# bhavyageethika/multimodal_autonomous_driving_perception_and_planning

Hardware: AMD Instinct MI355X
Metric: end-to-end frames/sec (1280x720 synthetic) (higher is better)
Workload: dtype f64; 1 GPU; config4: 64 stream(s)/GPU x 1-frame window per step, 1280x720, simulated detection + IoU tracker + 6-state KF + 21-candidate planner, one launch per step, up to 4 consecutive steps in flight; streams_per_gpu=64, window=1, graph=False, taggers=False, allgather_track_tables=False, fused_step=True, overlapped_steps=4, steps_per_library_call=8, parallelism=stream-sharded x1

## Files before the change

multimodal_autonomous_driving_perception_and_planning_amd/csrc/kf.hip:

```cpp
#include "common.h"

namespace {

struct KfOut {
    double v[AV_VSTATE_DOUBLES];
};

struct Filter {
    double x[6];
    double P[6][6];
    double prev_heading, prev_speed, time;
};

__device__ __forceinline__ void extract(Filter& k, double dt, KfOut& o) {
    const double vx = k.x[2], vy = k.x[3];
    const double speed = sqrt(vx * vx + vy * vy);
    const double heading = speed > 0.1 ? atan2(vy, vx) : k.prev_heading;
    const double acc = dt > 0.0 ? (speed - k.prev_speed) / dt : 0.0;
    double dh = heading - k.prev_heading;
    const double pi = 3.141592653589793;
    if (dh > pi) dh -= 2.0 * pi;
    else if (dh < -pi) dh += 2.0 * pi;
    const double yaw = dt > 0.0 ? dh / dt : 0.0;
    o.v[0] = k.x[0], o.v[1] = k.x[1], o.v[2] = vx, o.v[3] = vy;
// ... 110 lines not shown
    double* st = kf_state + (size_t)s * AV_KF_STATE_DOUBLES;

    bool bad = st[45] != 0.0;
    if (lane < 36) {
        const int r = lane / 6, c = lane - r * 6;
        if (((r ^ c) & 1) && st[6 + lane] != 0.0) bad = true;
    }
    if (__ballot(bad) != 0ull) {
        if (lane == 0) st[45] = 1.0;
        return false;
    }
    const int ax = lane & 1;
    Axis a;
    a.x0 = st[ax], a.x1 = st[2 + ax], a.x2 = st[4 + ax];
#pragma unroll
    for (int r = 0; r < 3; ++r)
#pragma unroll
        for (int c = 0; c < 3; ++c) a.p[r][c] = st[6 + (2 * r + ax) * 6 + (2 * c + ax)];
    double carry_h = st[42], carry_sp = st[43], time = st[44];
    double pp[3][3], Kc[3][2] = {{0, 0}, {0, 0}, {0, 0}};
#pragma unroll
    for (int r = 0; r < 3; ++r)
#pragma unroll
        for (int c = 0; c < 3; ++c) pp[r][c] = a.p[r][c];
    bool steady = false;
    __builtin_amdgcn_s_waitcnt(0x0F70);
    const double dt = cfg.dt, h = 0.5 * (dt * dt), q = cfg.process_noise, rr = cfg.measurement_noise;

    for (int f0 = 0; f0 < n_frames; f0 += KF_BATCH) {
        const int nb = (n_frames - f0) < KF_BATCH ? (n_frames - f0) : KF_BATCH;
        const size_t sf0 = (size_t)s * n_frames + f0;
        int m_mine = 0;
        if (lane < nb) {
            const int m = mode ? (int)mode[sf0 + lane] : 1;
            m_mine = m;
            ml[lane] = m;
            double4 zz = make_double4(0.0, 0.0, 0.0, 0.0);
            if (z && (m == 1 || m == 3)) zz = reinterpret_cast<const double4*>(z)[sf0 + lane];
            *reinterpret_cast<double4*>(zl[lane]) = zz;
        }
        __builtin_amdgcn_s_waitcnt(0x0F70);
        __builtin_amdgcn_fence(__ATOMIC_RELEASE, "wavefront", "local");
        __builtin_amdgcn_wave_barrier();
        __builtin_amdgcn_fence(__ATOMIC_ACQUIRE, "wavefront", "local");

        const unsigned long long ones = __ballot(m_mine == 1);
        for (int fb = 0; fb < nb;) {
            if (steady) {
                const double p00 = a.p[0][0], p11 = a.p[1][1];
                while (fb < nb && ((ones >> fb) & 1ull)) {
                    const double zp = zl[fb][ax], zv = zl[fb][2 + ax];
                    const double nx0 = a.x0 + dt * a.x1 + h * a.x2;
                    const double nx1 = a.x1 + dt * a.x2;
                    a.x0 = nx0, a.x1 = nx1;
                    time += dt;
                    const double vpred = a.x1;
                    const double y0 = zp - a.x0, y1 = zv - a.x1;
                    a.x0 = a.x0 + (Kc[0][0] * y0 + Kc[0][1] * y1);
                    a.x1 = a.x1 + (Kc[1][0] * y0 + Kc[1][1] * y1);
                    a.x2 = a.x2 + (Kc[2][0] * y0 + Kc[2][1] * y1);
                    if (lane < 2) {
                        double* w = raw[fb];
                        w[ax] = a.x0, w[2 + ax] = a.x1, w[4 + ax] = vpred;
                        w[6 + ax] = p00, w[8 + ax] = p11;
                        if (lane == 0) w[10] = time, w[11] = 1.0;
                    }
                    ++fb;
                }
                if (fb >= nb) break;
            }
            const int m = ml[fb];
            const double zp = zl[fb][ax], zv = zl[fb][2 + ax];
            double vpred = a.x1;
            {
                if (m != 3) {
                    axis_predict(a, dt, h, q);
                    time += dt;
                    vpred = a.x1;
                }
                if (m == 1 || m == 3) axis_update(a, zp, zv, rr, Kc);
                bool same = m == 1;
#pragma unroll
                for (int r = 0; r < 3; ++r)
#pragma unroll
                    for (int c = 0; c < 3; ++c) same = same && a.p[r][c] == pp[r][c], pp[r][c] = a.p[r][c];
                steady = __ballot(same) == ~0ull;
            }
            if (lane < 2) {
                double* w = raw[fb];
                w[ax] = a.x0, w[2 + ax] = a.x1, w[4 + ax] = vpred;
                w[6 + ax] = a.p[0][0], w[8 + ax] = a.p[1][1];
                if (lane == 0) w[10] = time, w[11] = (double)m;
            }
            ++fb;
        }
        __builtin_amdgcn_fence(__ATOMIC_RELEASE, "wavefront", "local");
        __builtin_amdgcn_wave_barrier();
        __builtin_amdgcn_fence(__ATOMIC_ACQUIRE, "wavefront", "local");

        const bool on = lane < nb;
        const double* w = raw[on ? lane : 0];
        const int m = (int)w[11];
        const double px = w[0], py = w[1], vx = w[2], vy = w[3], vxp = w[4], vyp = w[5];
        const bool has_pred = (m != 3), has_post = (m == 1 || m == 3);
        const double sp_p = sqrt(vxp * vxp + vyp * vyp);
        const double sp_q = sqrt(vx * vx + vy * vy);
        const bool val_p = has_pred && sp_p > 0.1, val_q = has_post && sp_q > 0.1;
        const double at_p = atan2(vyp, vxp), at_q = atan2(vy, vx);
        const bool gives = on && (val_p || val_q);
        const double give_h = val_q ? at_q : at_p;
        const unsigned long long gmask = __ballot(gives);
        const unsigned long long below = gmask & ((1ull << lane) - 1ull);
        const int src = below ? 63 - __clzll((long long)below) : 0;
        const double from_h = __shfl(give_h, src, 64);
        const double h_in = below ? from_h : carry_h;
        const double last_sp = has_post ? sp_q : sp_p;
        double sp_in = __shfl_up(last_sp, 1, 64);
        if (lane == 0) sp_in = carry_sp;
        const double h_p = has_pred ? (val_p ? at_p : h_in) : h_in;
        const double prev_h = has_pred ? h_p : h_in;
        const double prev_s = has_pred ? sp_p : sp_in;
        double heading, speed, ph, ps;
        if (m == 0) heading = h_p, speed = sp_p, ph = h_in, ps = sp_in;
        else if (m == 2) heading = (sp_p > 0.1 ? at_p : prev_h), speed = sp_p, ph = prev_h, ps = prev_s;
        else heading = (val_q ? at_q : prev_h), speed = sp_q, ph = prev_h, ps = prev_s;
        const double acc = dt > 0.0 ? (speed - ps) / dt : 0.0;
        double dh = heading - ph;
        const double pi = 3.141592653589793;
        if (dh > pi) dh -= 2.0 * pi;
        else if (dh < -pi) dh += 2.0 * pi;
        const double yaw = dt > 0.0 ? dh / dt : 0.0;
        if (on) {
            double2* dst = reinterpret_cast<double2*>(out_state + (sf0 + lane) * AV_VSTATE_DOUBLES);
            dst[0] = make_double2(px, py), dst[1] = make_double2(vx, vy), dst[2] = make_double2(heading, speed);
            dst[3] = make_double2(acc, yaw), dst[4] = make_double2(w[10], sqrt(w[6] + w[7]));
            dst[5] = make_double2(sqrt(w[8] + w[9]), 0.0);
            if (plan_state) reinterpret_cast<double4*>(plan_state)[sf0 + lane] = make_double4(px, py, heading, speed);
        }
        carry_h = __shfl(heading, nb - 1, 64);
        carry_sp = __shfl(speed, nb - 1, 64);
    }

    if (lane < 2) {
        st[ax] = a.x0, st[2 + ax] = a.x1, st[4 + ax] = a.x2;
#pragma unroll
        for (int r = 0; r < 3; ++r)
#pragma unroll
            for (int c = 0; c < 3; ++c) st[6 + (2 * r + ax) * 6 + (2 * c + ax)] = a.p[r][c];
        if (lane == 0) st[42] = carry_h, st[43] = carry_sp, st[44] = time;
    }
    return true;
}

template <bool DENSE>
__global__ void __launch_bounds__(64) kf_axis_kernel(av_kf_cfg cfg, int n_frames, const double* __restrict__ z,
                                                     const uint8_t* __restrict__ mode, double* __restrict__ kf_state,
                                                     double* __restrict__ out_state, double* __restrict__ plan_state) {
    __builtin_amdgcn_s_setprio(3);
    const bool separable = kf_axis_body(cfg, n_frames, z, mode, kf_state, out_state, plan_state, blockIdx.x, threadIdx.x);
    if (DENSE && !separable && threadIdx.x == 0) kf_dense_stream_lds(cfg, blockIdx.x, n_frames, z, mode, kf_state, out_state, plan_state);
}

__global__ void kf_reset_kernel(int n_streams, double* kf_state) {
    const int s = blockIdx.x * blockDim.x + threadIdx.x;
    if (s >= n_streams) return;
    double* st = kf_state + (size_t)s * AV_KF_STATE_DOUBLES;
    for (int i = 0; i < AV_KF_STATE_DOUBLES; ++i) st[i] = 0.0;
    for (int i = 0; i < 6; ++i) st[6 + i * 7] = 10.0;
}

}

#ifndef AVHOT_DEVICE_ONLY

extern "C" {

int av_kf_reset(av_ctx* ctx, av_stream_t stream, int n_streams, double* kf_state) {
    AV_REQUIRE(ctx && kf_state && n_streams > 0, AV_EINVAL, "av_kf_reset: bad argument");
    hipLaunchKernelGGL(kf_reset_kernel, dim3((n_streams + 63) / 64), dim3(64), 0, as_stream(stream), n_streams, kf_state);
    AV_LAUNCH_CHECK();
    return AV_OK;
}

int av_kf_step(av_ctx* ctx, av_stream_t stream, const av_kf_cfg* cfg, int n_streams, int n_frames, const double* z,
               const uint8_t* mode, double* kf_state, double* out_state, double* plan_state) {
    AV_REQUIRE(ctx && cfg && kf_state && out_state, AV_EINVAL, "av_kf_step: null argument");
    AV_REQUIRE(z || mode, AV_EINVAL, "av_kf_step: z may only be NULL when every mode is 0 or 2");
    AV_REQUIRE(n_streams > 0 && n_frames > 0, AV_EINVAL, "av_kf_step: n_streams/n_frames must be > 0");
    if (n_frames <= 2) {
        hipLaunchKernelGGL(kf_axis_kernel<true>, dim3(n_streams), dim3(64), 0, as_stream(stream), *cfg, n_frames, z, mode, kf_state,
                           out_state, plan_state);
        AV_LAUNCH_CHECK();
        return AV_OK;
    }
    hipLaunchKernelGGL(kf_axis_kernel<false>, dim3(n_streams), dim3(64), 0, as_stream(stream), *cfg, n_frames, z, mode,
                       kf_state, out_state, plan_state);
    AV_LAUNCH_CHECK();
    hipLaunchKernelGGL(kf_kernel, dim3((n_streams + 63) / 64), dim3(64), 0, as_stream(stream), *cfg, n_streams,
                       n_frames, z, mode, kf_state, out_state, plan_state, 1);
    AV_LAUNCH_CHECK();
    return AV_OK;
}

}

#endif
```

multimodal_autonomous_driving_perception_and_planning_amd/csrc/planner.hip:

```cpp
#include "common.h"

#include <cmath>



namespace {

struct PlanParams {
    int n, n_lat, C;
    double dt, H;
    double w_lat, w_vel, w_acc, w_curv;
    const double *t, *alpha, *q, *dtd, *lat;
    double atq[20];
};

static const double ATAN_Q[20] = {
    -0x1.5555555555549p-2, 0x1.99999999979b9p-3,  -0x1.24924923e22b4p-3, 0x1.c71c718e5a102p-4,
    -0x1.745d120df88fbp-4, 0x1.3b1362fc35ab5p-4,  -0x1.110deef367776p-4, 0x1.e1b3c8d50e91fp-5,
    -0x1.ae2c7119eb922p-5, 0x1.81fdd2525246ap-5,  -0x1.56daf4786fd80p-5, 0x1.2575526b2309ap-5,
    -0x1.d168e01adf666p-6, 0x1.462cc26bda000p-6,  -0x1.8055065b73333p-7, 0x1.693bd6b79999ap-8,
    -0x1.fdf4e15cccccdp-10, 0x1.f224118000000p-12, -0x1.2568700000000p-14, 0x1.2ed799999999ap-18,
};

__device__ __forceinline__ double atan2_fast(double y, double x, const double (&Q)[20]) {
    const double ax = __builtin_fabs(x), ay = __builtin_fabs(y);
    const bool swap = ay > ax;
    const double mx = swap ? ay : ax, mn = swap ? ax : ay;
    double r = __builtin_amdgcn_rcp(mx);
    r = __builtin_fma(__builtin_fma(-mx, r, 1.0), r, r);
    r = __builtin_fma(__builtin_fma(-mx, r, 1.0), r, r);
    double t = mn * r;
    t = __builtin_fma(__builtin_fma(-t, mx, mn), r, t);
    t = mx == 0.0 ? 0.0 : t;
    const double z = t * t;
    double pz = Q[19];
#pragma unroll
    for (int k = 18; k >= 0; --k) pz = __builtin_fma(pz, z, Q[k]);
    double a = __builtin_fma(t * z, pz, t);
    a = swap ? 1.5707963267948966 - a : a;
    a = x < 0.0 ? 3.141592653589793 - a : a;
    return __builtin_copysign(a, y);
}

__host__ __device__ inline int even_up(int v) { return (v + 1) & ~1; }

__host__ __device__ inline size_t plan_lds_doubles(int G, int n, int C, int NW = 4) {
    return (size_t)G * 3 * n * 2 + even_up(G * 3 * 3) + (size_t)G * 8 + (size_t)3 * even_up(G * C) + (size_t)NW * n * 6;
}

__device__ __forceinline__ void wave_lds_fence() {
    __builtin_amdgcn_fence(__ATOMIC_RELEASE, "wavefront", "local");
    __builtin_amdgcn_wave_barrier();
    __builtin_amdgcn_fence(__ATOMIC_ACQUIRE, "wavefront", "local");
}

template <int G, int NW>
__device__ __forceinline__ void plan_block(const PlanParams& p, int f0, int n_states, const double* __restrict__ state,
                                           const double* __restrict__ ref, int n_ref, const double* __restrict__ obs, int n_obs,
                                           double* __restrict__ wp, double* __restrict__ cost, int32_t* __restrict__ order, double* sm) {
    const int n = p.n, C = p.C;
    double* vs = sm;
    double* base = vs + (size_t)G * 3 * n * 2;
    double* trig = base + even_up(G * 3 * 3);
    double* costs = trig + G * 8;
    double* stage_all = costs + 3 * even_up(G * C);
    const int CS = even_up(G * C);

    const int tid = threadIdx.x, lane = tid & 63, wid = tid >> 6;
    double* stage = stage_all + (size_t)wid * n * 6;
    constexpr int P = G * 3;
    static_assert(NW >= 2, "the heading terms take the last wave");

    auto bcast = [&](double x, int i) {
        const unsigned lo = (unsigned)__builtin_amdgcn_readlane((int)(unsigned)__double_as_longlong(x), i);
        const unsigned hi = (unsigned)__builtin_amdgcn_readlane((int)(unsigned)((unsigned long long)__double_as_longlong(x) >> 32), i);
        return __longlong_as_double((long long)(((unsigned long long)hi << 32) | lo));
    };
    auto terms = [&](double v0, double dv, int i, double& v, double& vdt, double& velt, double& acct) {
        v = v0 + dv * p.alpha[i];
        vdt = v * p.dt;
        const double e = v - 10.0;
        velt = p.w_vel * (e * e);
        acct = 0.0;
        if (i > 0) {
            const double vp = v0 + dv * p.alpha[i - 1];
            const double a = (v - vp) / p.dtd[i];
            acct = p.w_acc * (a * a);
        }
    };
    auto cost_chains = [&](double velt, double acct, unsigned long long hasm, double* b) {
        double sv = 0.0;
#pragma unroll
        for (int i = 0; i < 64; ++i)
            if (i < n) sv = sv + bcast(velt, i);
        double run = sv, sa = 0.0;
#pragma unroll
        for (int i = 1; i < 64; ++i)
            if (i < n && ((hasm >> i) & 1ull)) {
                const double term = bcast(acct, i);
                run = run + term, sa = sa + term;
            }
        if (lane == 0) b[0] = sv, b[1] = sa, b[2] = run;
    };

    const bool fast = n <= 64 && P <= NW;
    double k_velt = 0.0, k_acct = 0.0;
    unsigned long long k_has = 0;
    bool k_live = false;
    if (fast) {
        if (wid < P) {
            const int g = wid / 3, k = wid - g * 3, f = f0 + g;
            if (f < n_states) {
                const double v0 = state[(size_t)f * 4 + 3];
                const double vt = 8.0 + 2.0 * (double)k;
                const double dv = vt - v0;
                double* o = vs + ((size_t)(g * 3 + k) * n) * 2;
                double v = 0.0, vdt = 0.0;
                bool has = false;
                if (lane < n) terms(v0, dv, lane, v, vdt, k_velt, k_acct), has = lane > 0 && p.dtd[lane] > 0.0;
                k_has = __ballot(has), k_live = true;
                double sacc = 0.0, my_s = 0.0;
#pragma unroll
                for (int i = 1; i < 64; ++i)
                    if (i < n) {
                        sacc = sacc + bcast(vdt, i);
                        my_s = lane == i ? sacc : my_s;
                    }
                if (lane < n) o[2 * lane] = v, o[2 * lane + 1] = my_s;
            }
        }
    } else {
        for (int pr = wid; pr < P; pr += NW) {
            const int g = pr / 3, k = pr - g * 3, f = f0 + g;
            if (f >= n_states) continue;
            const double v0 = state[(size_t)f * 4 + 3];
            const double vt = 8.0 + 2.0 * (double)k;
            const double dv = vt - v0;
            double* o = vs + ((size_t)(g * 3 + k) * n) * 2;
            double* b = base + (g * 3 + k) * 3;
            double* tv = stage;
            for (int i = lane; i < n; i += 64) {
                double v, vdt, velt, acct;
                terms(v0, dv, i, v, vdt, velt, acct);
                o[2 * i] = v, tv[i] = vdt, tv[n + i] = velt, tv[2 * n + i] = acct;
            }
            wave_lds_fence();
            if (lane == 0) {
                double sacc = 0.0, sv = 0.0;
                o[1] = 0.0;
                sv = sv + tv[n];
                for (int i = 1; i < n; ++i) {
                    sacc = sacc + tv[i];
                    o[2 * i + 1] = sacc;
                    sv = sv + tv[n + i];
                }
                double run = sv, sa = 0.0;
                for (int i = 1; i < n; ++i) {
                    if (p.dtd[i] > 0.0) {
                        const double term = tv[2 * n + i];
                        run = run + term, sa = sa + term;
                    }
                }
                b[0] = sv, b[1] = sa, b[2] = run;
            }
            wave_lds_fence();
        }
    }
    if (wid == NW - 1 && lane < 2 * G) {
        const int g = lane >> 1, f = f0 + g;
        if (f < n_states) {
            const double h0 = state[(size_t)f * 4 + 2];
            double* tg = trig + g * 8;
            double sn, cs;
            if (lane & 1) {
                sincos(h0 + 1.5707963267948966, &sn, &cs);
                tg[4] = cs, tg[5] = sn;
            } else {
                sincos(h0, &sn, &cs);
                tg[0] = state[(size_t)f * 4 + 0], tg[1] = state[(size_t)f * 4 + 1];
                tg[2] = cs, tg[3] = sn, tg[6] = h0;
            }
        }
    }
    __syncthreads();
    if (k_live) cost_chains(k_velt, k_acct, k_has, base + wid * 3);

    const double q_l = lane < n ? p.q[lane] : 0.0, q_l1 = lane + 1 < n ? p.q[lane + 1] : 0.0, t_l = lane < n ? p.t[lane] : 0.0;
    const bool extra = n_ref > 0 || n_obs > 0;
    for (int j = fast ? (wid - P % NW + NW) % NW : wid; j < G * C; j += NW) {
        const int g = j / C, c = j - g * C, f = f0 + g;
        if (f >= n_states) continue;
        const int li = c / 3, k = c - li * 3;
        const double df = p.lat[li];
        const double* tg = trig + g * 8;
        const double x0 = tg[0], y0 = tg[1], cs = tg[2], sn = tg[3], c2 = tg[4], s2 = tg[5], h0 = tg[6];
        const double* o = vs + ((size_t)(g * 3 + k) * n) * 2;

        for (int i = lane; i < n; i += 64) {
            const double v = o[2 * i], s = o[2 * i + 1];
            const bool first = i == lane;
            const double d = df * (first ? q_l : p.q[i]);
            double x = x0 + s * cs, y = y0 + s * sn;
            x = x + d * c2, y = y + d * s2;
            double hd = 0.0;
            if (i < n - 1) {
                const double s1 = o[2 * i + 3], d1 = df * (first ? q_l1 : p.q[i + 1]);
                double x1 = x0 + s1 * cs, y1 = y0 + s1 * sn;
                x1 = x1 + d1 * c2, y1 = y1 + d1 * s2;
                hd = atan2_fast(y1 - y, x1 - x, p.atq);
            }
            double* w = stage + (size_t)i * 6;
            w[0] = x, w[1] = y, w[2] = hd, w[3] = v, w[4] = first ? t_l : p.t[i], w[5] = 0.0;
        }
        wave_lds_fence();
        double lat_sum = 0.0, curv_sum = 0.0, obs_sum = 0.0;
        for (int i = lane; i < n; i += 64) {
            double* w = stage + (size_t)i * 6;
            double curv = 0.0;
            if (i > 0 && i < n - 1) {
                const double hp = stage[(size_t)(i - 1) * 6 + 2];
                curv = (w[2] - hp) / (w[3] * p.dt + 1e-6);
                w[5] = curv;
            }
            curv_sum += p.w_curv * (curv * curv);
            const double x = w[0], y = w[1];
            if (n_ref > 0) {
                double md = INFINITY;
                for (int r = 0; r < n_ref; ++r) {
                    const double dx = ref[2 * r] - x, dy = ref[2 * r + 1] - y;
                    const double dd = sqrt(dx * dx + dy * dy);
                    md = dd < md ? dd : md;
                }
                lat_sum += p.w_lat * (md * md);
            }
            for (int q = 0; q < n_obs; ++q) {
                const double ox = obs[3 * q], oy = obs[3 * q + 1], rad = obs[3 * q + 2];
                const double ex = x - ox, ey = y - oy;
                const double dist = sqrt(ex * ex + ey * ey);
                if (dist < rad * 2.0) obs_sum += 1000.0 * (rad * 2.0 - dist);
                else if (dist < rad * 4.0) obs_sum += 10.0 / (dist - rad + 0.1);
            }
        }
        wave_lds_fence();
        if (lane == 0) stage[(size_t)(n - 1) * 6 + 2] = n > 1 ? stage[(size_t)(n - 2) * 6 + 2] : h0;
        curv_sum = wave_sum_dpp(curv_sum);
        if (extra) lat_sum = wave_sum_dpp(lat_sum), obs_sum = wave_sum_dpp(obs_sum);
        if (lane == 0) costs[g * C + c] = lat_sum, costs[CS + g * C + c] = curv_sum, costs[2 * CS + g * C + c] = obs_sum;
        wave_lds_fence();
        if (wp) {
            const double2* src = reinterpret_cast<const double2*>(stage);
            double2* dst = reinterpret_cast<double2*>(wp + ((size_t)f * C + c) * n * 6);
            for (int q = lane; q < n * 3; q += 64) dst[q] = src[q];
        }
        wave_lds_fence();
    }
    __syncthreads();

    for (int idx = tid; idx < G * C; idx += NW * 64) {
        const int g = idx / C, c = idx - g * C, k = c % 3;
        const double* b = base + (g * 3 + k) * 3;
        const double va = n_ref > 0 ? (costs[idx] + b[0]) + b[1] : b[2];
        const double total = (va + costs[CS + idx]) + costs[2 * CS + idx];
        costs[idx] = total;
    }
    __syncthreads();
    for (int idx = tid; idx < G * C; idx += NW * 64) {
        const int g = idx / C, c = idx - g * C, f = f0 + g;
        if (f >= n_states) continue;
        const double* cc = costs + g * C;
        const double mine = cc[c];
        int rank = 0;
        for (int o2 = 0; o2 < C; ++o2) {
            const double v = cc[o2];
            rank += (v < mine || (v == mine && o2 < c)) ? 1 : 0;
        }
        cost[(size_t)f * C + c] = mine;
        order[(size_t)f * C + rank] = c;
    }
}

template <int G, int NW>
__global__ void __launch_bounds__(NW * 64) planner_kernel(PlanParams p, int n_states, const double* __restrict__ state,
                                                          const double* __restrict__ ref, int n_ref,
                                                          const double* __restrict__ obs, int n_obs,
                                                          double* __restrict__ wp, double* __restrict__ cost,
                                                          int32_t* __restrict__ order) {
    extern __shared__ __attribute__((aligned(16))) double sm[];
    plan_block<G, NW>(p, blockIdx.x * G, n_states, state, ref, n_ref, obs, n_obs, wp, cost, order, sm);
}

constexpr int RING_UNITS = 256, RING_DOUBLES = RING_UNITS * 2;

template <int FPW, bool EXTRA>
__global__ void __launch_bounds__(256) planner_wave_kernel(PlanParams p, int n_states,
                                                           const double* __restrict__ state,
                                                           const double* __restrict__ ref, int n_ref,
                                                           const double* __restrict__ obs, int n_obs,
                                                           double* __restrict__ wp, double* __restrict__ cost,
                                                           int32_t* __restrict__ order) {
    extern __shared__ __attribute__((aligned(16))) double sm[];
    const int n = p.n, C = p.C;
    const int lane = threadIdx.x & 63, wid = threadIdx.x >> 6;
    const size_t per_wave = (size_t)FPW * 3 * n * 2 + RING_DOUBLES + even_up(FPW * C) + FPW * 3 * 4 + FPW * 8;
    double* vs = sm + wid * per_wave;
    double* stage = vs + (size_t)FPW * 3 * n * 2;
    double* costs = stage + RING_DOUBLES;
    double* base = costs + even_up(FPW * C);
    double* trig = base + FPW * 3 * 4;
    const long long gw = (long long)blockIdx.x * 4 + wid;
    const long long f0l = gw * FPW;
    if (f0l >= n_states) return;
    const int f0 = (int)f0l;
    const int nf = (n_states - f0) < FPW ? (n_states - f0) : FPW;

    const bool in = lane < n;
    const int li_c = in ? lane : n - 1;
    const int ln_c = (lane + 1 < n) ? lane + 1 : n - 1;
    const int lp_c = li_c > 0 ? li_c - 1 : 0;
    const double q_i = p.q[li_c], q_n = p.q[ln_c], t_i = p.t[li_c];
    const double al_i = p.alpha[li_c], al_p = p.alpha[lp_c], dtd_i = p.dtd[li_c];
    const double lat_l = p.lat[lane < p.n_lat ? lane : 0];
    double st_x[FPW], st_y[FPW], st_h[FPW], st_v[FPW];
#pragma unroll
    for (int g = 0; g < FPW; ++g) {
        const double4 sv4 = reinterpret_cast<const double4*>(state)[f0 + (g < nf ? g : 0)];
        st_x[g] = sv4.x, st_y[g] = sv4.y, st_h[g] = sv4.z, st_v[g] = sv4.w;
    }

#pragma unroll
    for (int g = 0; g < FPW; ++g) {
        if (g < nf) {
#pragma unroll
            for (int k = 0; k < 3; ++k) {
                const int pair = g * 3 + k;
                const double v0 = st_v[g];
                const double dv = (8.0 + 2.0 * (double)k) - v0;
                const double v = v0 + dv * al_i;
                const double vp = v0 + dv * al_p;
// ... 410 lines not shown
```

multimodal_autonomous_driving_perception_and_planning_amd/csrc/step.hip:

```cpp
#define AVHOT_DEVICE_ONLY
#include "simdet.hip"
#include "tracker.hip"
#include "kf.hip"
#include "planner.hip"
#undef AVHOT_DEVICE_ONLY

namespace {

struct StepArgs {
    int S, h, w, dcap, tcap;
    av_tracker_cfg tcfg;
    av_kf_cfg kcfg;
    PlanParams pp;
    int32_t* frame_count; const SimRow* tab; const double* cdf;
    int32_t *det_n, *det_box, *det_cls; double* det_conf; int32_t* det_status;
    unsigned char* trk_state; av_track_row* snap; int32_t* snap_n; int32_t* det2trk;
    const double* z; double *kf_state, *vstate, *plan_state;
    double *wp, *cost; int32_t* order;
    uint8_t* wire; int stream0, frame0;
    int* flags; int seq, spin, fence, stage_off;
};

constexpr int STEP_NW = 8;

__device__ __host__ inline int flag_fault(int S) { return 64 * S; }
__device__ __host__ inline int flag_base(int S) { return 64 * S + 32; }
__device__ __host__ inline int flag_stats(int S) { return 65 * S + 32; }
struct StepClock {
    unsigned long long t;
    bool on;
    unsigned long long* acc;
    __device__ void start(const StepArgs& a, int role);
    __device__ void mark(int k) {
        if (!on) return;
        const unsigned long long n = __builtin_amdgcn_s_memrealtime();
        atomicAdd(acc + k, n - t);
        t = n;
    }
};

__device__ void StepClock::start(const StepArgs& a, int role) {
    on = a.flags && (a.fence & 8) && threadIdx.x == 0;
    if (!on) return;
    acc = reinterpret_cast<unsigned long long*>(a.flags + flag_stats(a.S)) + role * 16;
    t = __builtin_amdgcn_s_memrealtime();
    atomicAdd(acc + 15, 1ull);
}

__device__ __forceinline__ bool seq_enter(const StepArgs& a, int slot, int* go) {
    if (threadIdx.x == 0) {
        int ok = 0;
        int* const counter = a.flags + 32 * slot;
        int* const fault = a.flags + flag_fault(a.S);
        const int want = a.seq, spin = a.spin;
        for (int n = 0; n <= spin; ++n) {
            if ((int)((unsigned)__hip_atomic_load(counter, __ATOMIC_RELAXED, __HIP_MEMORY_SCOPE_AGENT) - (unsigned)want) >= 0) { ok = 1; break; }
            if ((n & 255) == 255 && __hip_atomic_load(fault, __ATOMIC_RELAXED, __HIP_MEMORY_SCOPE_AGENT) != 0) break;
        }
        if (!ok) atomicOr(a.flags + flag_fault(a.S), 1);
        if (ok && (a.fence & 8) && a.seq != 0) {
            const unsigned long long tp = __hip_atomic_load(reinterpret_cast<unsigned long long*>(a.flags + 32 * slot + 2), __ATOMIC_RELAXED,
                                                            __HIP_MEMORY_SCOPE_AGENT);
            const unsigned long long now = __builtin_amdgcn_s_memrealtime();
            unsigned long long* acc = reinterpret_cast<unsigned long long*>(a.flags + flag_stats(a.S)) + (slot & 1) * 16;
            if (now > tp) atomicAdd(acc + 8, now - tp), atomicAdd(acc + 9, 1ull);
        }
        *go = ok;
    }
    __syncthreads();
    if (!*go) return false;
    if (a.fence & 1) __builtin_amdgcn_fence(__ATOMIC_ACQUIRE, "agent");
    return true;
}
__device__ __forceinline__ void seq_leave(const StepArgs& a, int slot) {
    if (a.fence & 2) __builtin_amdgcn_fence(__ATOMIC_RELEASE, "agent");
    if (a.fence & 8)
        __hip_atomic_store(reinterpret_cast<unsigned long long*>(a.flags + 32 * slot + 2), __builtin_amdgcn_s_memrealtime(), __ATOMIC_RELAXED,
                           __HIP_MEMORY_SCOPE_AGENT);
    __hip_atomic_store(a.flags + 32 * slot, (int)((unsigned)a.seq + 1u), __ATOMIC_RELAXED, __HIP_MEMORY_SCOPE_AGENT);
}
__device__ __forceinline__ void fetch_record(const void* src, void* dst_lds, int n8, int first, int end, bool coherent) {
    unsigned long long* g = const_cast<unsigned long long*>(reinterpret_cast<const unsigned long long*>(src));
    unsigned long long* l = reinterpret_cast<unsigned long long*>(dst_lds);
    if ((int)threadIdx.x < first || (int)threadIdx.x >= end) return;
    for (int i = (int)threadIdx.x - first; i < n8; i += end - first)
        l[i] = coherent ? __hip_atomic_load(g + i, __ATOMIC_RELAXED, __HIP_MEMORY_SCOPE_AGENT) : g[i];
}

template <int PW>
__global__ void __launch_bounds__(PW * 64) hot_step_kernel(StepArgs a) {
    extern __shared__ __attribute__((aligned(16))) unsigned char smem[];
    __shared__ int go, fc_stage;
    __shared__ __attribute__((aligned(16))) double kf_stage[AV_KF_STATE_DOUBLES + 2];
    __shared__ __attribute__((aligned(16))) int d_box[8 * 4];
    __shared__ __attribute__((aligned(16))) double d_conf[8], d_area[8], z_stage[4];
    __shared__ int d_cls[8], d_n[1];
    const int tid = threadIdx.x;
    const bool seq = a.flags != nullptr;
    if ((int)blockIdx.x < a.S) {
        if (PW > STEP_NW && tid >= STEP_NW * 64) return;
        const int s = blockIdx.x;
        StepClock ck;
        ck.start(a, 0);
        int fc_before = 0;
        if (tid == 0) {
            fc_before = seq ? (int)((unsigned)a.flags[flag_base(a.S) + s] + (unsigned)a.seq) : a.frame_count[s];
            fc_stage = fc_before;
            simdet_frame<true>(0, 0, 0, a.h, a.w, a.dcap, &fc_stage, a.tab, a.cdf, d_n, d_box, d_cls, d_conf,
                               a.det_status ? a.det_status + s : nullptr);
            for (int i = 0; i < a.dcap; ++i)
                d_area[i] = (double)(d_box[4 * i + 2] - d_box[4 * i]) * (double)(d_box[4 * i + 3] - d_box[4 * i + 1]);
        }
        ck.mark(0);
        if (seq && !seq_enter(a, 2 * s, &go)) return;
        ck.mark(1);
        unsigned char* stage = smem + a.stage_off;
        int fc0 = 0;
        if (seq && tid == 0) fc0 = __hip_atomic_load(a.frame_count + s, __ATOMIC_RELAXED, __HIP_MEMORY_SCOPE_AGENT);
        fetch_record(a.trk_state + (size_t)s * state_bytes(a.tcap, a.tcfg.trajectory_length), stage,
                     (HDR_INTS * 4 + a.tcap * (int)sizeof(av_track_row)) / 8, 64, STEP_NW * 64, seq);
        if (tid == 0) {
            if (seq) {
                if (fc0 != fc_before) atomicOr(a.flags + flag_fault(a.S), 2);
                __hip_atomic_store(a.frame_count + s, fc_stage, __ATOMIC_RELAXED, __HIP_MEMORY_SCOPE_AGENT);
            } else {
                a.frame_count[s] = fc_stage;
            }
        }
        if (seq) __builtin_amdgcn_s_waitcnt(0x0F70);
        __syncthreads();
        ck.mark(2);
        if (tid < a.dcap) {
            reinterpret_cast<int4*>(a.det_box)[(size_t)s * a.dcap + tid] = reinterpret_cast<const int4*>(d_box)[tid];
            a.det_cls[(size_t)s * a.dcap + tid] = d_cls[tid];
            a.det_conf[(size_t)s * a.dcap + tid] = d_conf[tid];
            if (tid == 0) a.det_n[s] = d_n[0];
        }
        tracker_body<false, 8, STEP_NW>(a.tcfg, 1, a.dcap, d_n, d_box, d_cls, d_conf, a.tcap, a.trk_state, a.snap, a.snap_n,
                                        a.det2trk, 1, s, smem, 0xFEDCBA9876543210ull, stage, seq, 0,
                                        seq ? a.flags + 32 * (2 * s) : nullptr, (int)((unsigned)a.seq + 1u), (a.fence & 8) != 0, d_area);
        ck.mark(3);
        if (a.wire) {
            __syncthreads();
            if (tid < a.tcap)
                wire_put(a.wire + (size_t)s * (AV_WIRE_HDR_BYTES + (size_t)a.tcap * AV_WIRE_ROW_BYTES), tid, a.snap_n[s], a.tcap,
                         a.snap + (size_t)s * a.tcap, a.stream0 + s, a.frame0 + fc_stage);
        }
    } else {
        const int s = blockIdx.x - a.S;
        StepClock ck;
        ck.start(a, 1);
        if (tid < 4) z_stage[tid] = a.z[(size_t)s * 4 + tid];
        if (seq && !seq_enter(a, 2 * s + 1, &go)) return;
        ck.mark(1);
        if (tid < 64) {
            double* rec = a.kf_state + (size_t)s * AV_KF_STATE_DOUBLES;
            fetch_record(rec, kf_stage, AV_KF_STATE_DOUBLES, 0, 64, seq);
            __builtin_amdgcn_fence(__ATOMIC_RELEASE, "workgroup", "local");
            __builtin_amdgcn_wave_barrier();
            __builtin_amdgcn_fence(__ATOMIC_ACQUIRE, "workgroup", "local");
            ck.mark(2);
            const double* z = z_stage;
            double *vs = a.vstate + (size_t)s * AV_VSTATE_DOUBLES, *ps = a.plan_state + (size_t)s * 4;
            const bool separable = kf_axis_body(a.kcfg, 1, z, nullptr, kf_stage, vs, ps, 0, tid);
            if (!separable && tid == 0) kf_dense_stream_lds(a.kcfg, 0, 1, z, nullptr, kf_stage, vs, ps);
            __builtin_amdgcn_fence(__ATOMIC_RELEASE, "workgroup", "local");
            __builtin_amdgcn_wave_barrier();
            __builtin_amdgcn_fence(__ATOMIC_ACQUIRE, "workgroup", "local");
            if (tid < AV_KF_STATE_DOUBLES) {
                if (seq)
                    __hip_atomic_store(reinterpret_cast<unsigned long long*>(rec) + tid, (unsigned long long)__double_as_longlong(kf_stage[tid]),
                                       __ATOMIC_RELAXED, __HIP_MEMORY_SCOPE_AGENT);
                else
                    rec[tid] = kf_stage[tid];
            }
        }
        ck.mark(3);
        if (seq && tid < 64) {
            __builtin_amdgcn_s_waitcnt(0x0F70);
            if (tid == 0) seq_leave(a, 2 * s + 1);
        }
        ck.mark(4);
        __syncthreads();
        plan_block<1, PW>(a.pp, s, a.S, a.plan_state, nullptr, 0, nullptr, 0, a.wp, a.cost, a.order, reinterpret_cast<double*>(smem));
        ck.mark(6);
    }
}

}

static size_t hot_step_tracker_lds(int dcap, int tcap, int& stage_off) {
    static_assert(STEP_NW == 8, "tracker_lds_bytes sizes the replica kernel's eight column waves");
    const size_t lds_t = (tracker_lds_bytes(tcap, dcap, 1, true, 0) + 15) & ~size_t(15);
    stage_off = (int)lds_t;
    return lds_t + HDR_INTS * 4 + (size_t)tcap * sizeof(av_track_row);
}

static size_t hot_step_static_lds(const void* kernel) {
    hipFuncAttributes fa{};
    return hipFuncGetAttributes(&fa, kernel) == hipSuccess ? (size_t)fa.sharedSizeBytes : (size_t)16384;
}

static int hot_step_shape(const av_ctx* ctx, int n_streams, size_t lds_t, int depth, size_t& lds_out, int& pw_out) {
    static const size_t lds_static16 = hot_step_static_lds(reinterpret_cast<const void*>(hot_step_kernel<16>));
    static const size_t lds_static8 = hot_step_static_lds(reinterpret_cast<const void*>(hot_step_kernel<8>));
    const char* pwe = getenv("AVHOT_STEP_PW");
    int pw = pwe && atoi(pwe) == 8 ? 8 : 16;
    size_t lds = 0;
    for (;;) {
        const size_t lds_p = plan_lds_doubles(1, ctx->n_points, ctx->n_cand, pw) * 8;
        lds = lds_t > lds_p ? lds_t : lds_p;
        const size_t lds_static = pw == 16 ? lds_static16 : lds_static8;
        if (lds + lds_static > 64 * 1024) {
            AV_REQUIRE(pw == 16 && !pwe, AV_EINVAL,
                       "av_hot_step: configuration needs %zu B of dynamic + %zu B of static LDS (limit 65536)", lds, lds_static);
            pw = 8;
            continue;
        }
        if (depth <= 1) break;
        int per_cu = 0;
        if (pw == 16) AV_HIP(hipOccupancyMaxActiveBlocksPerMultiprocessor(&per_cu, hot_step_kernel<16>, 16 * 64, lds));
        else AV_HIP(hipOccupancyMaxActiveBlocksPerMultiprocessor(&per_cu, hot_step_kernel<8>, 8 * 64, lds));
        if ((long long)depth * 2 * n_streams <= (long long)per_cu * ctx->n_cus) break;
        AV_REQUIRE(pw == 16 && !pwe, AV_EINVAL, "av_hot_step: %d launches of %d workgroups in flight do not fit the device (%d per CU x %d CUs)",
                   depth, 2 * n_streams, per_cu, ctx->n_cus);
        pw = 8;
    }
    lds_out = lds, pw_out = pw;
    return AV_OK;
}

static int hot_step_args(av_ctx* ctx, const av_tracker_cfg* tcfg, const av_kf_cfg* kcfg, int n_streams, int h,
                           int w, int dcap, int tcap, int32_t* frame_count, int32_t* det_n, int32_t* det_box, int32_t* det_cls,
                           double* det_conf, int32_t* det_status, void* tracker_state, av_track_row* snap, int32_t* snap_n,
                           int32_t* det2trk, const double* z, double* kf_state, double* vstate, double* plan_state,
                           double* waypoints, double* cost, int32_t* order, void* wire, int stream0, int frame0, int32_t* seq_flags,
                           int seq, StepArgs& a, size_t& lds_out, int& pw_out, int depth = 1) {
    AV_REQUIRE(ctx && tcfg && kcfg && frame_count && det_n && det_box && det_cls && det_conf && tracker_state && z && kf_state &&
                   vstate && plan_state && cost && order,
               AV_EINVAL, "av_hot_step: null argument");
    AV_REQUIRE(n_streams > 0, AV_EINVAL, "av_hot_step: n_streams must be > 0");
    AV_REQUIRE(ctx->planner_ready && ctx->d_simtab, AV_ESTATE, "av_hot_step: call av_planner_configure first");
    AV_REQUIRE((snap == nullptr) == (snap_n == nullptr), AV_EINVAL, "av_hot_step: snap and snap_n go together");
    AV_REQUIRE(!wire || snap, AV_EINVAL, "av_hot_step: the wire tables are made from the snapshot rows");
    AV_REQUIRE(tcap == 64 && dcap >= 7 && dcap <= 8 && tcfg->iou_threshold > 0.0 && tcfg->trajectory_length >= 1, AV_EINVAL,
               "av_hot_step: needs tcap 64, dcap 7..8 and iou_threshold > 0 (use the stage calls otherwise)");
    AV_REQUIRE(h > 0 && w > 121, AV_EINVAL, "av_hot_step: frame %dx%d too small", w, h);
    a = StepArgs{};
    a.S = n_streams, a.h = h, a.w = w, a.dcap = dcap, a.tcap = tcap;
    a.tcfg = *tcfg, a.kcfg = *kcfg;
    fill_params(ctx, a.pp);
    a.frame_count = frame_count, a.tab = (const SimRow*)ctx->d_simtab, a.cdf = ctx->d_cdf;
    a.det_n = det_n, a.det_box = det_box, a.det_cls = det_cls, a.det_conf = det_conf, a.det_status = det_status;
    a.trk_state = (unsigned char*)tracker_state, a.snap = snap, a.snap_n = snap_n, a.det2trk = det2trk;
    a.z = z, a.kf_state = kf_state, a.vstate = vstate, a.plan_state = plan_state;
    a.wp = waypoints, a.cost = cost, a.order = order;
    a.wire = (uint8_t*)wire, a.stream0 = stream0, a.frame0 = frame0;
    a.flags = seq_flags, a.seq = seq;
    const char* spe = seq_flags ? getenv("AVHOT_STEP_SPIN") : nullptr;
    a.spin = spe ? atoi(spe) : (1 << 22);
    const char* fe = seq_flags ? getenv("AVHOT_STEP_FENCE") : nullptr;
    a.fence = fe ? atoi(fe) : 0;
    int stage_off = 0;
    const size_t lds_t = hot_step_tracker_lds(dcap, tcap, stage_off);
    a.stage_off = stage_off;
    return hot_step_shape(ctx, n_streams, lds_t, depth, lds_out, pw_out);
}

static int hot_step_go(const StepArgs& a, size_t lds, int pw, av_stream_t stream) {
    if (pw == 16) hipLaunchKernelGGL(hot_step_kernel<16>, dim3(2 * a.S), dim3(16 * 64), lds, as_stream(stream), a);
    else hipLaunchKernelGGL(hot_step_kernel<8>, dim3(2 * a.S), dim3(8 * 64), lds, as_stream(stream), a);
    AV_LAUNCH_CHECK();
    return AV_OK;
}

static int hot_step_launch(av_ctx* ctx, av_stream_t stream, const av_tracker_cfg* tcfg, const av_kf_cfg* kcfg, int n_streams, int h,
                           int w, int dcap, int tcap, int32_t* frame_count, int32_t* det_n, int32_t* det_box, int32_t* det_cls,
                           double* det_conf, int32_t* det_status, void* tracker_state, av_track_row* snap, int32_t* snap_n,
                           int32_t* det2trk, const double* z, double* kf_state, double* vstate, double* plan_state,
                           double* waypoints, double* cost, int32_t* order, void* wire, int stream0, int frame0, int32_t* seq_flags,
                           int seq, int depth = 1) {
    StepArgs a;
    size_t lds;
    int pw;
    const int rc = hot_step_args(ctx, tcfg, kcfg, n_streams, h, w, dcap, tcap, frame_count, det_n, det_box, det_cls, det_conf, det_status,
                                 tracker_state, snap, snap_n, det2trk, z, kf_state, vstate, plan_state, waypoints, cost, order, wire, stream0,
                                 frame0, seq_flags, seq, a, lds, pw, depth);
    return rc != AV_OK ? rc : hot_step_go(a, lds, pw, stream);
}

extern "C" int av_hot_step_fits(av_ctx* ctx, int n_streams, int dcap, int tcap, int depth) {
    AV_REQUIRE(ctx && n_streams > 0 && depth >= 1, AV_EINVAL, "av_hot_step_fits: bad argument");
    AV_REQUIRE(ctx->planner_ready, AV_ESTATE, "av_hot_step_fits: call av_planner_configure first");
    AV_REQUIRE(tcap == 64 && dcap >= 7 && dcap <= 8, AV_EINVAL, "av_hot_step_fits: needs tcap 64, dcap 7..8");
    AV_HIP(hipSetDevice(ctx->device));
    int stage_off = 0;
    size_t lds = 0;
    int pw = 0;
    return hot_step_shape(ctx, n_streams, hot_step_tracker_lds(dcap, tcap, stage_off), depth, lds, pw);
}

extern "C" int av_hot_step(av_ctx* ctx, av_stream_t stream, const av_tracker_cfg* tcfg, const av_kf_cfg* kcfg, int n_streams, int h,
                           int w, int dcap, int tcap, int32_t* frame_count, int32_t* det_n, int32_t* det_box, int32_t* det_cls,
                           double* det_conf, int32_t* det_status, void* tracker_state, av_track_row* snap, int32_t* snap_n,
                           int32_t* det2trk, const double* z, double* kf_state, double* vstate, double* plan_state,
                           double* waypoints, double* cost, int32_t* order, void* wire, int stream0, int frame0) {
    return hot_step_launch(ctx, stream, tcfg, kcfg, n_streams, h, w, dcap, tcap, frame_count, det_n, det_box, det_cls, det_conf, det_status,
                           tracker_state, snap, snap_n, det2trk, z, kf_state, vstate, plan_state, waypoints, cost, order, wire, stream0,
                           frame0, nullptr, 0);
}

extern "C" int av_hot_step_seq(av_ctx* ctx, av_stream_t stream, const av_tracker_cfg* tcfg, const av_kf_cfg* kcfg, int n_streams, int h,
                               int w, int dcap, int tcap, int32_t* frame_count, int32_t* det_n, int32_t* det_box, int32_t* det_cls,
                               double* det_conf, int32_t* det_status, void* tracker_state, av_track_row* snap, int32_t* snap_n,
                               int32_t* det2trk, const double* z, double* kf_state, double* vstate, double* plan_state,
                               double* waypoints, double* cost, int32_t* order, void* wire, int stream0, int frame0,
                               int32_t* seq_flags, int seq, int depth) {
    AV_REQUIRE(seq_flags, AV_EINVAL, "av_hot_step_seq: needs the sequence flags (AV_STEP_FLAG_INTS(n_streams) int32)");
    AV_REQUIRE(depth >= 2 && depth <= AV_STEP_MAX_DEPTH, AV_EINVAL, "av_hot_step_seq: depth %d not in [2, %d]", depth, AV_STEP_MAX_DEPTH);
    return hot_step_launch(ctx, stream, tcfg, kcfg, n_streams, h, w, dcap, tcap, frame_count, det_n, det_box, det_cls, det_conf, det_status,
                           tracker_state, snap, snap_n, det2trk, z, kf_state, vstate, plan_state, waypoints, cost, order, wire, stream0,
                           frame0, seq_flags, seq, depth);
}

extern "C" int av_hot_steps_seq(av_ctx* ctx, int depth, const av_stream_t* streams, const av_tracker_cfg* tcfg, const av_kf_cfg* kcfg,
                                int n_streams, int h, int w, int dcap, int tcap, int32_t* frame_count, int32_t* det_status,
                                void* tracker_state, double* kf_state, const av_step_set* sets, const double* z_steps, void* wire_steps,
                                int stream0, int frame0, int32_t* seq_flags, int seq0, int n_steps) {
    AV_REQUIRE(seq_flags && n_steps > 0 && sets && streams, AV_EINVAL, "av_hot_steps_seq: bad argument");
    AV_REQUIRE(depth >= 2 && depth <= AV_STEP_MAX_DEPTH, AV_EINVAL, "av_hot_steps_seq: depth %d not in [2, %d]", depth, AV_STEP_MAX_DEPTH);
    for (int k = 0; k < depth; ++k)
        for (int j = 0; j < k; ++j)
            AV_REQUIRE(streams[k] != streams[j], AV_EINVAL, "av_hot_steps_seq: the %d steps in flight need %d different HIP streams", depth, depth);
    StepArgs par[AV_STEP_MAX_DEPTH];
    size_t lds = 0;
    int pw = 16;
    for (int k = 0; k < depth; ++k) {
// ... 19 lines not shown
```

Baseline: 12.73 million frames/s.

## Split single-frame KF into critical chain and deferred tail overlapped with planner

For the one-frame step path, the Kalman filter is split into a short critical chain (predict/update, heading, start state written to LDS) and a tail (acceleration, yaw rate, covariance outputs, global vstate/plan_state writes). The planner now reads its start state directly from shared memory, and the tail runs on an idle planner wave after the first cost phase. The planner's wave-to-task mapping is rotated so that wave 0, which ran the KF, is free for the tail. This shortens the dependency between the KF and the planner and hides the output work. In exchange it adds a __syncthreads, more LDS, duplicated heading logic, and tighter coupling between the KF and the planner.

```diff
diff --git a/multimodal_autonomous_driving_perception_and_planning_amd/csrc/kf.hip b/multimodal_autonomous_driving_perception_and_planning_amd/csrc/kf.hip
--- a/multimodal_autonomous_driving_perception_and_planning_amd/csrc/kf.hip
+++ b/multimodal_autonomous_driving_perception_and_planning_amd/csrc/kf.hip
@@ -286,6 +286,90 @@
     return true;
 }
 
+__device__ __forceinline__ double kf_lane_bcast(double x, int i) {
+    const unsigned lo = (unsigned)__builtin_amdgcn_readlane((int)(unsigned)__double_as_longlong(x), i);
+    const unsigned hi = (unsigned)__builtin_amdgcn_readlane((int)(unsigned)((unsigned long long)__double_as_longlong(x) >> 32), i);
+    return __longlong_as_double((long long)(((unsigned long long)hi << 32) | lo));
+}
+
+constexpr int KF_CARRY_DOUBLES = 4;
+
+__device__ __forceinline__ bool kf_axis_chain1(const av_kf_cfg& cfg, const double* __restrict__ z, double* __restrict__ st,
+                                               double* __restrict__ start, double* __restrict__ carry, const int lane) {
+    bool bad = st[45] != 0.0;
+    if (lane < 36) {
+        const int r = lane / 6, c = lane - r * 6;
+        if (((r ^ c) & 1) && st[6 + lane] != 0.0) bad = true;
+    }
+    if (__ballot(bad) != 0ull) {
+        if (lane == 0) st[45] = 1.0;
+        return false;
+    }
+    const int ax = lane & 1;
+    Axis a;
+    a.x0 = st[ax], a.x1 = st[2 + ax], a.x2 = st[4 + ax];
+#pragma unroll
+    for (int r = 0; r < 3; ++r)
+#pragma unroll
+        for (int c = 0; c < 3; ++c) a.p[r][c] = st[6 + (2 * r + ax) * 6 + (2 * c + ax)];
+    const double h_in = st[42];
+    double time = st[44];
+    const double zp = z[ax], zv = z[2 + ax];
+    const double dt = cfg.dt, h = 0.5 * (dt * dt), q = cfg.process_noise, rr = cfg.measurement_noise;
+    axis_predict(a, dt, h, q);
+    time += dt;
+    const double vpred = a.x1;
+    double K[3][2];
+    axis_update(a, zp, zv, rr, K);
+    const double px = kf_lane_bcast(a.x0, 0), py = kf_lane_bcast(a.x0, 1), vx = kf_lane_bcast(a.x1, 0), vy = kf_lane_bcast(a.x1, 1);
+    const double sp_q = sqrt(vx * vx + vy * vy);
+    double heading;
+    if (sp_q > 0.1) {
+        heading = atan2(vy, vx);
+    } else {
+        const double vxp = kf_lane_bcast(vpred, 0), vyp = kf_lane_bcast(vpred, 1);
+        const double sp_p = sqrt(vxp * vxp + vyp * vyp);
+        heading = sp_p > 0.1 ? atan2(vyp, vxp) : h_in;
+    }
+    if (lane < 2) {
+        st[ax] = a.x0, st[2 + ax] = a.x1, st[4 + ax] = a.x2;
+#pragma unroll
+        for (int r = 0; r < 3; ++r)
+#pragma unroll
+            for (int c = 0; c < 3; ++c) st[6 + (2 * r + ax) * 6 + (2 * c + ax)] = a.p[r][c];
+        carry[ax] = vpred;
+        if (lane == 0) {
+            st[42] = heading, st[43] = sp_q, st[44] = time;
+            carry[2] = h_in;
+            start[0] = px, start[1] = py, start[2] = heading, start[3] = sp_q;
+        }
+    }
+    return true;
+}
+
+__device__ __forceinline__ void kf_axis_tail1(const av_kf_cfg& cfg, const double* __restrict__ st, const double* __restrict__ carry,
+                                              double* __restrict__ out_state, double* __restrict__ plan_state, const int lane) {
+    const double dt = cfg.dt;
+    const double px = st[0], py = st[1], vx = st[2], vy = st[3], heading = st[42], speed = st[43];
+    const double vxp = carry[0], vyp = carry[1], h_in = carry[2];
+    const double sp_p = sqrt(vxp * vxp + vyp * vyp);
+    const double at_p = atan2(vyp, vxp);
+    const double h_p = sp_p > 0.1 ? at_p : h_in;
+    const double acc = dt > 0.0 ? (speed - sp_p) / dt : 0.0;
+    double dh = heading - h_p;
+    const double pi = 3.141592653589793;
+    if (dh > pi) dh -= 2.0 * pi;
+    else if (dh < -pi) dh += 2.0 * pi;
+    const double yaw = dt > 0.0 ? dh / dt : 0.0;
+    if (lane == 0) {
+        double2* dst = reinterpret_cast<double2*>(out_state);
+        dst[0] = make_double2(px, py), dst[1] = make_double2(vx, vy), dst[2] = make_double2(heading, speed);
+        dst[3] = make_double2(acc, yaw), dst[4] = make_double2(st[44], sqrt(st[6] + st[13]));
+        dst[5] = make_double2(sqrt(st[20] + st[27]), 0.0);
+        if (plan_state) *reinterpret_cast<double4*>(plan_state) = make_double4(px, py, heading, speed);
+    }
+}
+
 template <bool DENSE>
 __global__ void __launch_bounds__(64) kf_axis_kernel(av_kf_cfg cfg, int n_frames, const double* __restrict__ z,
                                                      const uint8_t* __restrict__ mode, double* __restrict__ kf_state,
diff --git a/multimodal_autonomous_driving_perception_and_planning_amd/csrc/planner.hip b/multimodal_autonomous_driving_perception_and_planning_amd/csrc/planner.hip
--- a/multimodal_autonomous_driving_perception_and_planning_amd/csrc/planner.hip
+++ b/multimodal_autonomous_driving_perception_and_planning_amd/csrc/planner.hip
@@ -54,11 +54,17 @@
     __builtin_amdgcn_fence(__ATOMIC_ACQUIRE, "wavefront", "local");
 }
 
-template <int G, int NW>
+struct PlanNoHook {
+    __device__ __forceinline__ void operator()(int) const {}
+};
+
+template <int G, int NW, class Hook = PlanNoHook>
 __device__ __forceinline__ void plan_block(const PlanParams& p, int f0, int n_states, const double* __restrict__ state,
                                            const double* __restrict__ ref, int n_ref, const double* __restrict__ obs, int n_obs,
-                                           double* __restrict__ wp, double* __restrict__ cost, int32_t* __restrict__ order, double* sm) {
+                                           double* __restrict__ wp, double* __restrict__ cost, int32_t* __restrict__ order, double* sm,
+                                           int state_f0 = -1, int rot = 0, Hook after1 = Hook()) {
     const int n = p.n, C = p.C;
+    const int sd = state_f0 < 0 ? 0 : state_f0 - f0;
     double* vs = sm;
     double* base = vs + (size_t)G * 3 * n * 2;
     double* trig = base + even_up(G * 3 * 3);
@@ -66,8 +72,9 @@
     double* stage_all = costs + 3 * even_up(G * C);
     const int CS = even_up(G * C);
 
-    const int tid = threadIdx.x, lane = tid & 63, wid = tid >> 6;
-    double* stage = stage_all + (size_t)wid * n * 6;
+    const int tid = threadIdx.x, lane = tid & 63;
+    double* stage = stage_all + (size_t)(tid >> 6) * n * 6;
+    const int wid = ((tid >> 6) + NW - rot) % NW;
     constexpr int P = G * 3;
     static_assert(NW >= 2, "the heading terms take the last wave");
 
@@ -111,7 +118,7 @@
         if (wid < P) {
             const int g = wid / 3, k = wid - g * 3, f = f0 + g;
             if (f < n_states) {
-                const double v0 = state[(size_t)f * 4 + 3];
+                const double v0 = state[(size_t)(f + sd) * 4 + 3];
                 const double vt = 8.0 + 2.0 * (double)k;
                 const double dv = vt - v0;
                 double* o = vs + ((size_t)(g * 3 + k) * n) * 2;
@@ -133,7 +140,7 @@
         for (int pr = wid; pr < P; pr += NW) {
             const int g = pr / 3, k = pr - g * 3, f = f0 + g;
             if (f >= n_states) continue;
-            const double v0 = state[(size_t)f * 4 + 3];
+            const double v0 = state[(size_t)(f + sd) * 4 + 3];
             const double vt = 8.0 + 2.0 * (double)k;
             const double dv = vt - v0;
             double* o = vs + ((size_t)(g * 3 + k) * n) * 2;
@@ -169,7 +176,7 @@
     if (wid == NW - 1 && lane < 2 * G) {
         const int g = lane >> 1, f = f0 + g;
         if (f < n_states) {
-            const double h0 = state[(size_t)f * 4 + 2];
+            const double h0 = state[(size_t)(f + sd) * 4 + 2];
             double* tg = trig + g * 8;
             double sn, cs;
             if (lane & 1) {
@@ -177,13 +184,14 @@
                 tg[4] = cs, tg[5] = sn;
             } else {
                 sincos(h0, &sn, &cs);
-                tg[0] = state[(size_t)f * 4 + 0], tg[1] = state[(size_t)f * 4 + 1];
+                tg[0] = state[(size_t)(f + sd) * 4 + 0], tg[1] = state[(size_t)(f + sd) * 4 + 1];
                 tg[2] = cs, tg[3] = sn, tg[6] = h0;
             }
         }
     }
     __syncthreads();
     if (k_live) cost_chains(k_velt, k_acct, k_has, base + wid * 3);
+    after1(wid);
 
     const double q_l = lane < n ? p.q[lane] : 0.0, q_l1 = lane + 1 < n ? p.q[lane + 1] : 0.0, t_l = lane < n ? p.t[lane] : 0.0;
     const bool extra = n_ref > 0 || n_obs > 0;
diff --git a/multimodal_autonomous_driving_perception_and_planning_amd/csrc/step.hip b/multimodal_autonomous_driving_perception_and_planning_amd/csrc/step.hip
--- a/multimodal_autonomous_driving_perception_and_planning_amd/csrc/step.hip
+++ b/multimodal_autonomous_driving_perception_and_planning_amd/csrc/step.hip
@@ -92,6 +92,9 @@
     extern __shared__ __attribute__((aligned(16))) unsigned char smem[];
     __shared__ int go, fc_stage;
     __shared__ __attribute__((aligned(16))) double kf_stage[AV_KF_STATE_DOUBLES + 2];
+    __shared__ __attribute__((aligned(32))) double kf_start[4];
+    __shared__ __attribute__((aligned(16))) double kf_carry[KF_CARRY_DOUBLES];
+    __shared__ int kf_tail;
     __shared__ __attribute__((aligned(16))) int d_box[8 * 4];
     __shared__ __attribute__((aligned(16))) double d_conf[8], d_area[8], z_stage[4];
     __shared__ int d_cls[8], d_n[1];
@@ -153,6 +156,7 @@
         if (tid < 4) z_stage[tid] = a.z[(size_t)s * 4 + tid];
         if (seq && !seq_enter(a, 2 * s + 1, &go)) return;
         ck.mark(1);
+        double *vs = a.vstate + (size_t)s * AV_VSTATE_DOUBLES, *ps = a.plan_state + (size_t)s * 4;
         if (tid < 64) {
             double* rec = a.kf_state + (size_t)s * AV_KF_STATE_DOUBLES;
             fetch_record(rec, kf_stage, AV_KF_STATE_DOUBLES, 0, 64, seq);
@@ -160,10 +164,14 @@
             __builtin_amdgcn_wave_barrier();
             __builtin_amdgcn_fence(__ATOMIC_ACQUIRE, "workgroup", "local");
             ck.mark(2);
-            const double* z = z_stage;
-            double *vs = a.vstate + (size_t)s * AV_VSTATE_DOUBLES, *ps = a.plan_state + (size_t)s * 4;
-            const bool separable = kf_axis_body(a.kcfg, 1, z, nullptr, kf_stage, vs, ps, 0, tid);
-            if (!separable && tid == 0) kf_dense_stream_lds(a.kcfg, 0, 1, z, nullptr, kf_stage, vs, ps);
+            const bool separable = kf_axis_chain1(a.kcfg, z_stage, kf_stage, kf_start, kf_carry, tid);
+            if (tid == 0) {
+                kf_tail = separable;
+                if (!separable) {
+                    kf_dense_stream_lds(a.kcfg, 0, 1, z_stage, nullptr, kf_stage, vs, kf_start);
+                    *reinterpret_cast<double4*>(ps) = *reinterpret_cast<const double4*>(kf_start);
+                }
+            }
             __builtin_amdgcn_fence(__ATOMIC_RELEASE, "workgroup", "local");
             __builtin_amdgcn_wave_barrier();
             __builtin_amdgcn_fence(__ATOMIC_ACQUIRE, "workgroup", "local");
@@ -176,13 +184,25 @@
             }
         }
         ck.mark(3);
+        __syncthreads();
+        ck.mark(4);
+        constexpr int KF_ROT = 4;
+        static_assert(KF_ROT + 3 < PW, "wave 0 must not be a phase-1 pair wave nor the heading wave (task wave PW - 1)");
         if (seq && tid < 64) {
             __builtin_amdgcn_s_waitcnt(0x0F70);
             if (tid == 0) seq_leave(a, 2 * s + 1);
         }
-        ck.mark(4);
-        __syncthreads();
-        plan_block<1, PW>(a.pp, s, a.S, a.plan_state, nullptr, 0, nullptr, 0, a.wp, a.cost, a.order, reinterpret_cast<double*>(smem));
+        ck.mark(5);
+        const bool clocks = seq && (a.fence & 8);
+        auto tail = [&](int task_wave) {
+            if (task_wave != 0 || !kf_tail) return;
+            const unsigned long long t0 = clocks ? __builtin_amdgcn_s_memrealtime() : 0ull;
+            kf_axis_tail1(a.kcfg, kf_stage, kf_carry, vs, ps, tid & 63);
+            if (clocks && (tid & 63) == 0)
+                atomicAdd(reinterpret_cast<unsigned long long*>(a.flags + flag_stats(a.S)) + 16 + 7, __builtin_amdgcn_s_memrealtime() - t0);
+        };
+        plan_block<1, PW>(a.pp, s, a.S, kf_start, nullptr, 0, nullptr, 0, a.wp, a.cost, a.order, reinterpret_cast<double*>(smem), 0, KF_ROT,
+                          tail);
         ck.mark(6);
     }
 }
```

Result: faster. 13.45 million frames/s, median of 6 (+5.7%).
